# Gnnng/SVDFeature

Hardware: AMD Instinct MI355X
Metric: training instances/sec (SGD updates/s), basicMF k=64 (higher is better)
Workload: dtype f32; 1 GPU; basicMF synthetic 1000000x100000, 100000000 ratings, k=64 fp32 (BASELINE configs[1]); order=uniform random (file order preserved: result == sequential SGD), conflict_free_batches_per_pass=903, parallelism=1 GPU

## Files before the change

svdfeature_amd/csrc/svdf_capi.cpp:

```cpp
#include <svdfeature_amd.h>

#include <algorithm>
#include <cstdlib>
#include <cstring>
#include <new>
#include <vector>

#include "svdf_engine.h"
#include "svdf_kernels.h"
#include "svdf_wseq_rule.h"

namespace svdf {
void rank_eval_metrics(long S, const int64_t *sec_ptr, const int *position, const int *ranked, const int *nan, int num_at, const int *at,
                       svdf_rank_metrics *out);
void set_error_mode(int m);
const char *last_error();
void note_error(const std::string &m);
}

struct svdf_trainer { svdf::Engine *e; };
struct svdf_dataset { svdf::Dataset *d; };
struct svdf_ranker { svdf::Ranker *r; };

#define SVDF_GUARD(retval, ...)                                 \
// ... 212 lines not shown
int svdf_rank_prefetch_buffer_file(svdf_trainer *t, const char *path) { SVDF_GUARD(-1, { t->e->rank_prefetch(path); return 0; }) }
int64_t svdf_rank_sample_buffer_file(svdf_trainer *t, const char *in_path, const char *out_path) {
    SVDF_GUARD(-1, { return (int64_t)t->e->rank_sample_buffer_file(in_path, out_path); })
}
void svdf_dataset_destroy(svdf_dataset *ds) {
    if (!ds) return;
    try { if (ds->d && ds->d->owner) ds->d->owner->synchronize(); } catch (...) {}
    delete ds->d;
    delete ds;
}
int svdf_train_dataset(svdf_trainer *t, svdf_dataset *ds) { SVDF_GUARD(-1, { t->e->train_dataset(ds->d); return 0; }) }
int svdf_predict_dataset(svdf_trainer *t, svdf_dataset *ds, float *out) { SVDF_GUARD(-1, { t->e->predict_dataset(ds->d, out); return 0; }) }
int64_t svdf_dataset_info(const svdf_dataset *ds, int what) {
    if (!ds || !ds->d) return -1;
    switch (what) {
    case 0: return ds->d->num_row;
    case 1: return ds->d->kind == 8 ? (int64_t)ds->d->wchild.size() : (int64_t)ds->d->sched.num_levels();
    case 2: return ds->d->sched.max_level_size;
    case 3: return ds->d->kind;
    case 4: return ds->d->algorithmic_bytes;
    case 5: return ds->d->num_units;
    case 6: return ds->d->num_simple_units;
    case 7: {
        uint64_t h = 1469598103934665603ull;
        auto mix = [&h](uint64_t v) { for (int b = 0; b < 8; b++) { h ^= (v >> (8 * b)) & 0xFFu; h *= 1099511628211ull; } };
        for (long v : ds->d->sched.level_ptr) mix((uint64_t)v);
        for (long v : ds->d->sched.level_mid) mix((uint64_t)v);
        for (int v : ds->d->sched.order) mix((uint64_t)(unsigned)v);
        return (int64_t)(h >> 1);
    }
    case 8: return ds->d->kind == 8 && !ds->d->wchild.empty() ? (int64_t)ds->d->wchild[0]->kind : -1;
    case 9: return ds->d->rn_stage_state;
    case 10: return ds->d->rn_stage_bytes;
    default: return -1;
    }
}

int svdf_item_delta_begin(svdf_trainer *t) { SVDF_GUARD(-1, { t->e->per_rank_api(); t->e->item_delta_begin(); return 0; }) }
void *svdf_item_delta_buffer(svdf_trainer *t, int64_t *count) { SVDF_GUARD(nullptr, { t->e->per_rank_api(); return t->e->item_delta_buffer(count); }) }
int svdf_item_delta_apply(svdf_trainer *t) { SVDF_GUARD(-1, { t->e->per_rank_api(); t->e->item_delta_apply(); return 0; }) }
int svdf_item_delta_export(svdf_trainer *t, float *dst) { SVDF_GUARD(-1, { t->e->per_rank_api(); t->e->item_delta_copy(dst, nullptr); return 0; }) }
int svdf_item_delta_import(svdf_trainer *t, const float *src) { SVDF_GUARD(-1, { t->e->per_rank_api(); t->e->item_delta_copy(nullptr, src); return 0; }) }

int svdf_item_delta_into(svdf_trainer *t, float *dst, int64_t *count) { SVDF_GUARD(-1, { t->e->per_rank_api(); t->e->item_delta_into(dst, count); return 0; }) }
int svdf_item_delta_pack(svdf_trainer *t, void *dst, int half, int64_t *count) { SVDF_GUARD(-1, { t->e->per_rank_api(); t->e->item_delta_pack(dst, half, count); return 0; }) }
int svdf_item_delta_unpack(svdf_trainer *t, const void *src, int half, int refresh_snapshot) {
    SVDF_GUARD(-1, { t->e->per_rank_api(); t->e->item_delta_unpack(src, half, refresh_snapshot); return 0; })
}
int svdf_item_delta_select(svdf_trainer *t, int part, int nparts) { SVDF_GUARD(-1, { t->e->per_rank_api(); t->e->item_delta_select(part, nparts); return 0; }) }
int svdf_item_delta_apply_from(svdf_trainer *t, const float *src) { SVDF_GUARD(-1, { t->e->per_rank_api(); t->e->item_delta_apply_from(src); return 0; }) }
int svdf_set_stream(svdf_trainer *t, void *hip_stream) { SVDF_GUARD(-1, { t->e->set_stream((hipStream_t)hip_stream); return 0; }) }

int64_t svdf_get_view(svdf_trainer *t, int which, float *out, int64_t capacity) { SVDF_GUARD(-1, { return t->e->get_view(which, out, capacity); }) }
int64_t svdf_set_view(svdf_trainer *t, int which, const float *in, int64_t count) { SVDF_GUARD(-1, { return t->e->set_view(which, in, count); }) }
int svdf_view_shape(svdf_trainer *t, int which, int *rows, int *cols) { SVDF_GUARD(-1, { t->e->view_shape(which, rows, cols); return 0; }) }
void *svdf_stream(svdf_trainer *t) { return (void *)t->e->stream(); }
int svdf_synchronize(svdf_trainer *t) { SVDF_GUARD(-1, { t->e->synchronize(); return 0; }) }
int64_t svdf_counter(svdf_trainer *t, int what) { return t->e->counter(what); }
int svdf_set_knob(svdf_trainer *t, const char *name, long value) { SVDF_GUARD(-1, { return t->e->set_knob(name, value); }) }

int svdf_eval_dataset(svdf_trainer *t, svdf_dataset *ds, float scale_score, double *sum_sq_err, int64_t *count) {
    SVDF_GUARD(-1, { t->e->eval_dataset(ds->d, scale_score, sum_sq_err, count); return 0; })
}

int svdf_rank_eval_positions(svdf_trainer *t, long num_section, const unsigned *user, const int64_t *pos_ptr, const unsigned *pos_item,
                             const int64_t *ban_ptr, const unsigned *ban_item, int *position_out, int *tied_out, int *ranked_out, int *nan_out) {
// ... 117 lines not shown
```

svdfeature_amd/csrc/svdf_config.cpp:

```cpp
#include "svdf_engine.h"

#include <algorithm>
#include <chrono>
#include <cmath>
#include <cstdlib>
#include <cstring>
#include <memory>
#include <mutex>
#include <atomic>
#include <thread>

#include "svdf_kernels.h"
#include "svdf_internal.h"

namespace svdf {

void ParamSet::set_param(const char *name, const char *val) {
    if (!strncmp(name, prefix_a.c_str(), prefix_a.size())) name += prefix_a.size();
    else if (!strncmp(name, prefix_b.c_str(), prefix_b.size())) name += prefix_b.size();
    else return;
    if (!strcmp("bound", name)) {
        unsigned bd = (unsigned)atoi(val);
        check(bd > 0, "can't give 0 as bound");
        check(bound.empty() || bound.back() < bd, "bound must be given in order");
// ... 182 lines not shown
    case 38: return n_rank_eval_sections_;
    case 39: return n_rank_topn_sections_;
    case 21: return 0;
    default: return -1;
    }
}
int Engine::set_knob(const char *name, long value) {
    launch_version_++;
    if (multi_ && !is_peer_ && strcmp(name, "stage_window") != 0 && strcmp(name, "async_flush") != 0)
        for (int d = 1; d < gpus_; d++) (void)rank_engine(d)->set_knob(name, value);
    if (!strcmp(name, "use_graph")) { use_graph_ = value != 0; return 0; }
    if (!strcmp(name, "stage_window")) { check(value >= 1, "stage_window must be >= 1"); stage_window_ = value; window_set_ = true; return 0; }
    if (!strcmp(name, "groups_per_wave")) {
        check(value >= 0 && value <= 8 && value != 7, "groups_per_wave must be 0 (auto), 1 ... 6 or 8");
        groups_per_wave_ = (int)value;
        return 0;
    }
    if (!strcmp(name, "xcd_remap")) { xcd_remap_ = value != 0; params_dirty_ = true; return 0; }
    if (!strcmp(name, "fewrow_i16")) { check(value >= 0 && value <= 1, "fewrow_i16 must be 0 or 1"); fewrow_i16_ = (int)value; params_dirty_ = true; return 0; }
    if (!strcmp(name, "svdpp_helpers")) { check(value == 1 || value == 4 || value == 8 || value == 16, "svdpp_helpers must be 1, 4, 8 or 16"); svdpp_helpers_ = (int)value; params_dirty_ = true; return 0; }
    if (!strcmp(name, "basic_i8")) { check(value >= 0 && value <= 1, "basic_i8 must be 0 or 1"); basic_i8_ = (int)value; params_dirty_ = true; return 0; }
    if (!strcmp(name, "load_mode")) { check(value >= 0 && value <= 2, "load_mode must be 0, 1 or 2 (auto)"); load_mode_ = (int)value; params_dirty_ = true; return 0; }
    if (!strcmp(name, "store_mode")) { check(value >= 0 && value <= 2, "store_mode must be 0, 1 or 2"); store_mode_ = (int)value; params_dirty_ = true; return 0; }
    if (!strcmp(name, "sort_batches")) { check(value >= 0 && value <= 2, "sort_batches must be 0, 1 (by item) or 2 (by user)"); sort_batches_ = (int)value; return 0; }
    if (!strcmp(name, "async_flush")) { flush(); async_flush_ = value != 0; return 0; }
    if (!strcmp(name, "use_fused")) { use_fused_ = value != 0; return 0; }
    if (!strcmp(name, "device_schedule")) { device_sched_ = value != 0; return 0; }
    if (!strcmp(name, "device_rank")) { device_rank_ = value != 0; return 0; }
    if (!strcmp(name, "device_init")) { device_init_ = value != 0; return 0; }
    if (!strcmp(name, "device_window")) { device_window_ = value != 0; return 0; }
    if (!strcmp(name, "device_load")) { device_load_ = value != 0; return 0; }
    if (!strcmp(name, "runs_exec")) { check(value == 0 || value == 1, "runs_exec must be 0 or 1"); runs_exec_ = (int)value; return 0; }
    if (!strcmp(name, "runs_len")) { check(value >= 2 && value <= 7, "runs_len must be in 2 .. 7"); runs_len_ = (int)value; return 0; }
    if (!strcmp(name, "runs_sets")) { check(value >= 1 && value <= 2, "runs_sets must be 1 or 2"); runs_sets_ = (int)value; return 0; }
    if (!strcmp(name, "runs_block")) { check(value == 64 || value == 128 || value == 256, "runs_block must be 64, 128 or 256"); runs_block_ = (int)value; return 0; }
    if (!strcmp(name, "runs_min_rows")) { check(value >= 0, "runs_min_rows must not be negative"); runs_min_rows_ = value; return 0; }
    if (!strcmp(name, "runs_stage")) { check(value == 0 || value == 1, "runs_stage must be 0 or 1"); runs_stage_ = (int)value; return 0; }
    if (!strcmp(name, "runs_stage_max_mb")) { check(value >= -1, "runs_stage_max_mb must be -1 (no cap) or a size in MB"); runs_stage_max_mb_ = value; return 0; }
    if (!strcmp(name, "pair_units")) { check(value == 0 || value == 1, "pair_units must be 0 or 1"); pair_units_ = (int)value; return 0; }
    if (!strcmp(name, "pair_unit_cap")) { check(value >= 1 && value <= 4096, "pair_unit_cap must be in 1 .. 4096"); pair_unit_cap_ = (int)value; return 0; }
    if (!strcmp(name, "pivot_exec")) { check(value == 0 || value == 1, "pivot_exec must be 0 or 1"); pivot_exec_ = (int)value; return 0; }
    if (!strcmp(name, "pivot_run")) { check(value >= 1 && value <= 65536, "pivot_run must be in 1 .. 65536"); pivot_run_ = (int)value; return 0; }
    if (!strcmp(name, "pivot_min")) { check(value >= 2, "pivot_min must be at least 2"); pivot_min_ = (int)value; return 0; }
    if (!strcmp(name, "ipc_spin_limit")) { ipc_set_spin_limit(value); return 0; }
    if (!strcmp(name, "chain_width")) { check(value >= 0, "chain_width must not be negative"); chain_width_ = value; return 0; }
    if (!strcmp(name, "device_init_margin_log2")) { check(value >= 8 && value <= 52, "device_init_margin_log2 must be in 8 .. 52"); device_init_margin_log2_ = (int)value; return 0; }
    if (!strcmp(name, "device_schedule_min")) { check(value >= 1, "device_schedule_min must be >= 1"); device_sched_min_ = value; return 0; }
    if (!strcmp(name, "use_simple_units")) { use_simple_units_ = value != 0; return 0; }
    if (!strcmp(name, "rows_without_feedback")) { rows_without_feedback_ = value != 0; return 0; }
    if (!strcmp(name, "fewrow_gslots")) { fewrow_gslots_ = value != 0; launch_version_++; return 0; }
    if (!strcmp(name, "staged_pool")) { check(value == 0 || value == 1, "staged_pool must be 0 or 1"); flush(); staged_pool_mode_ = (int)value; return 0; }
    if (!strcmp(name, "wunit_inplace")) { wunit_inplace_ = value != 0; return 0; }
    if (!strcmp(name, "wunit_defer_fb")) { wunit_defer_fb_ = value != 0; return 0; }
    if (!strcmp(name, "wunit_fast")) { check(value >= 0 && value <= 3, "wunit_fast must be 0, 1, 2 or 3"); wunit_fast_ = (int)value; return 0; }
    if (!strcmp(name, "window_per_target_child")) { check(value >= 1, "window_per_target_child must be positive"); wseq_per_target_child_ = (int)value; return 0; }
    if (!strcmp(name, "window_per_target_shared")) { check(value >= 1, "window_per_target_shared must be positive"); wseq_per_target_shared_ = (int)value; return 0; }
    if (!strcmp(name, "window_per_target_fb")) { check(value >= 1, "window_per_target_fb must be positive"); wseq_per_target_fb_ = (int)value; return 0; }
    if (!strcmp(name, "window_shared_sub")) { check(value >= 0 && value <= 4096, "window_shared_sub must be in 0 .. 4096"); wseq_shared_sub_ = (int)value; return 0; }
    if (!strcmp(name, "window_shared_max")) { check(value >= 1, "window_shared_max must be positive"); wseq_shared_max_ = (int)value; return 0; }
    if (!strcmp(name, "window_item_sub")) { check(value >= 0 && value <= 128, "window_item_sub must be in 0 .. 128"); wseq_item_sub_ = (int)value; return 0; }
    if (!strcmp(name, "window_item_max")) { check(value >= 1, "window_item_max must be positive"); wseq_item_max_ = (int)value; return 0; }
    if (!strcmp(name, "window_block_sub")) {
        check(value >= 0 && value <= 4096, "window_block_sub must be in 0 .. 4096");
        check(value == 0 || (gpus_ == 1 && !multi_ && !is_peer_),
              "window_block_sub > 0 (ordered sub-steps for hot shared user rows of SVD++ blocks) is for the one-GPU window sequence; the N-rank exchange (amd:gpus > 1) has no place for user rows");
        wseq_block_sub_ = (int)value;
// ... 38 lines not shown
```

svdfeature_amd/csrc/svdf_dataset.cpp:

```cpp
#include "svdf_engine.h"

#include <algorithm>
#include <chrono>
#include <cmath>
#include <cstdlib>
#include <cstring>
#include <memory>
#include <mutex>
#include <atomic>
#include <thread>

#include "svdf_kernels.h"
#include "svdf_internal.h"

namespace svdf {

Dataset *Engine::dataset_from_blocks(long num_block, const int *extend_tag, const int64_t *fb_ptr, const unsigned *fb_index, const float *fb_value,
                                     const int64_t *block_row_ptr, const float *row_label, const int64_t *row_ptr, const unsigned *feat_index,
                                     const float *feat_value) {
    check(trainer_ready_, "dataset: init_trainer has not been called");
    need_device("dataset");
    check(user_group(), "svdfeature_amd: block datasets are for user-group (format_type 1) trainers");
    if (multi_ && !in_multi_scope()) {
        check(mp_.common_feedback_space == 0, "svdfeature_amd: amd:gpus > 1 needs a feedback space of its own (common_feedback_space = 0)");
// ... 534 lines not shown
    return true;
}
Dataset *Engine::auto_step(Dataset *exact, bool window_ok, const std::function<Dataset *()> &build_window) {
    std::unique_ptr<Dataset> ex(exact);
    AutoDecision D;
    double unit_us = 4.5;
    const bool from_probe = !ex;
    if (from_probe) { D = auto_probe_; D.decided = 0; }
    else auto_measures(ex.get(), D.levels, unit_us, D.dag_ms, D.stream_ms, pivot_run_);
    const bool deep = D.dag_ms > 2.0 * D.stream_ms;
    const char *why;
    if (!deep) { D.decided = 1; why = "exact levels kept (wide enough to stream)"; }
    else if (!window_ok) { D.decided = 3; why = "exact levels kept: the dependency depth binds, but the window step does not cover this configuration / these rows"; }
    else { D.decided = 2; why = "window step chosen: the dependency depth of exact sequential semantics binds"; }
    Dataset *out = ex.get();
    if (D.decided == 2) {
        ex.reset();
        out = build_window();
        D.windows = (long)out->wchild.size();
    } else {
        ex.release();
    }
    auto_last_ = D;
    if (!getenv("SVDF_QUIET"))
        fprintf(stderr, "[svdfeature_amd] amd:step = auto: %ld rows, %s%ld conflict-free levels: dag bound %.2f ms, stream model %.2f ms -> %s%s\n",
                (long)out->num_row, from_probe ? "extrapolated from the first 2 M rows: ~" : "", D.levels, D.dag_ms, D.stream_ms, why,
                D.decided == 2 ? (" (" + std::to_string(D.windows) + " windows)").c_str() : "");
    return out;
}

std::string Engine::path_for(const Dataset *ds) const {
    const DevParams &P = const_cast<Engine *>(this)->params();
    const long L = (long)ds->sched.num_levels();
    char buf[512];
    auto levels = [&](const char *what) { snprintf(buf, sizeof(buf), "exact, %ld conflict-free levels: %s", L, what); return std::string(buf); };
    switch (ds->kind) {
    case 0: return levels(chain_width_ > 0 ? "contract kernel k_basicmf / k_basicmf_slots, one (user, item) instance per lane group; narrow levels chained (k_basicmf_slots_chain)"
                                           : "contract kernel k_basicmf / k_basicmf_slots, one (user, item) instance per lane group");
    case 1: return levels("general sparse kernel k_general (any number of ids per row, side tables, lazy decay)");
    case 2: {
        const FusedSchedule S = ds->fused.view();
        if (fewrow_gslots_ && fewrow_fast_ && fewrow_gslots_applies(P, S, ds->fused.max_nu, ds->fused.max_ni, ds->fused.dense_slots))
            return levels("few-row kernel with global ids k_fewrow_gslots (neighbourhood shape)");
        return levels(fewrow_fast_ && fewrow_fast_applies(P, S) ? "few-row kernel k_fewrow_slots (<= 2 user + 2 item rows per instance: rank pairs, side ids); narrow levels chained"
                                                                 : "fused few-row kernel k_fused");
    }
    case 3: snprintf(buf, sizeof(buf), "exact, %ld conflict-free levels of user units: k_svdpp_wave (one wave per user, %ld of %ld units) + k_svdpp (general units)",
                     L, ds->num_simple_units, ds->num_units); return buf;
    case 4: return levels("multi-level implicit feedback units k_imfb");
    case 5: return "window data set (one window of the window-minibatch step, user side exact): k_window_users / k_window_items";
    case 6: return "amd:gpus handle: per-rank windows (svdf_multi.cpp)";
    case 7: return "window data set of user units: k_wunit_* (svdf_k_wunit.hip)";
    case 8: snprintf(buf, sizeof(buf), "window sequence (amd:step = minibatch / auto): %zu windows, each trained and applied in place%s%s; NOT the reference's sequential semantics (|dRMSE| <= 1e-4 contract)",
                     ds->wchild.size(), side_tables() ? ", feature_user / feature_item children as shared rows (general walk k_wunit_walk)" : "",
                     !ds->wchild.empty() && ds->wchild[0]->kind == 7 && !wunit_width_ok() ? ", user units of wide rows: the wide general walk k_wunit_walk<64, ., ., WideRow>, one wave per unit" : ""); return buf;
    case 9: snprintf(buf, sizeof(buf), "exact, %ld levels: hot rows walked as units (k_svdpp_wave on %s parameters, %ld units) + cold ratings through the contract kernel",
                     L, ds->pv_item_pivot ? "transposed" : "plain", ds->num_units); return buf;
    case 10: {
        char st[96] = "rows in W";
        if (runs_staged(ds)) snprintf(st, sizeof(st), "rows handed from run to run through staging slots (runs_stage, %.1f MB)", (double)ds->rn_stage_bytes / 1048576.0);
        else if (ds->rn_stage_state == 2) snprintf(st, sizeof(st), "rows in W (operand staging refused)");
        snprintf(buf, sizeof(buf), "exact, %ld levels of runs: k_basicmf_runs_soa (up to %d consecutive ratings of one item per lane group, the item's row in registers); %s", L, ds->rn_len, st);
        return buf;
    }
    case 11: snprintf(buf, sizeof(buf), "exact, %ld levels of user-run units: k_pair_units (%ld units of up to %d consecutive pairs of one user, the user's row in registers)",
                      L, ds->num_units, pair_unit_cap_); return buf;
    default: return "unknown";
    }
}
void Engine::note_dataset(Dataset *ds) {
    if (!ds || host_only_ || is_peer_) return;
    const bool verbose = getenv("SVDF_VERBOSE") != nullptr, quiet = getenv("SVDF_QUIET") != nullptr;
    if (verbose && !quiet) fprintf(stderr, "[svdfeature_amd] data set of %ld rows -> %s\n", (long)ds->num_row, path_for(ds).c_str());
    if (step_auto_set_ || step_minibatch_set_ || multi_ || gpus_ != 1) return;
    if (!(ds->kind == 0 || ds->kind == 1 || ds->kind == 2 || ds->kind == 3 || ds->kind == 4 || ds->kind == 9 || ds->kind == 10 || ds->kind == 11) || ds->num_row <= 0) return;
    AutoDecision D;
    double unit_us = 4.5;
    auto_measures(ds, D.levels, unit_us, D.dag_ms, D.stream_ms, pivot_run_);
    guard_last_ = D;
    if (D.dag_ms <= 10.0 * D.stream_ms || D.dag_ms < 50.0) return;
    n_guard_warnings_++;
    if (quiet) return;
    const bool window_ok = ds->plain_rows ? wunit_config_ok(false) && window_rows_allowed() && (wseq_pair_sub_ == 0 || wunit_width_ok())
                                          : wunit_config_ok() && (ds->kind == 3 || ds->kind == 4 || basic_fast_path_allowed());
    fprintf(stderr, "[svdfeature_amd] default (exact) step: %ld rows in %ld conflict-free levels -- the data's dependency depth binds: about %.0f ms per pass "
                    "(%.2f M rows/s; levels x %.1f us) against %.1f ms if the rows streamed.  The exact pass keeps the reference's sequential result bit for bit; "
                    "%s\n",
            (long)ds->num_row, D.levels, D.dag_ms, (double)ds->num_row / D.dag_ms * 1e-3, unit_us, D.stream_ms,
            window_ok ? "`amd:step = auto` would train this data set with the window step (user side exact, shared rows once per window; |dRMSE| <= 1e-4 contract) near the streaming rate"
                      : "the window step of `amd:step = auto` does not cover this configuration");
}

Dataset::~Dataset() {
    for (auto &per_rank : mchild) for (Dataset *c : per_rank) delete c;
    for (Dataset *c : wchild) delete c;
// ... 227 lines not shown
```

svdfeature_amd/csrc/svdf_engine.h:

```cpp
#ifndef SVDF_ENGINE_H_
#define SVDF_ENGINE_H_

#include <hip/hip_runtime.h>

#include <condition_variable>
#include <cstdio>
#include <memory>
#include <mutex>
#include <stdexcept>
#include <thread>
#include <string>
#include <deque>
#include <functional>
#include <future>
#include <map>
#include <vector>

#include "svdf_types.h"

namespace svdf {

struct Error : std::runtime_error {
    explicit Error(const std::string &m) : std::runtime_error(m) {}
};
// ... 196 lines not shown
    DevBuf<int> pos_list, neg_list;
    bool general = false;
    std::vector<int> h_tag;
    std::vector<int64_t> h_fb_ptr;
    std::vector<unsigned> h_fb_index;
    std::vector<float> h_fb_value;
    DevBuf<int> g_row_ptr, pair_p, pair_n, lens, optr;
    DevBuf<unsigned> g_index, out_index;
    DevBuf<float> g_value, out_label, out_value;
    void *scan_tmp = nullptr;
    size_t scan_tmp_bytes = 0;
    ~RankSource() { if (scan_tmp) (void)hipFree(scan_tmp); }
};
class Engine;
class Ranker;

struct Dataset {
    Engine *owner = nullptr;
    long num_row = 0;
    int kind = 0;
    DevBuf<WinUser> win_urec;
    DevBuf<int> win_slot, win_iptr, win_slot1;
    DevBuf<unsigned> win_item1;
    DevBuf<float> win_ival1;
    long win_item_lo = 0, win_item_hi = -1;
    DevBuf<long> d_level_ptr;
    bool d_level_ptr_ok = false;
    DevBuf<PairUnit> pu_units;
    DevBuf<unsigned> pu_lo, pu_hi;
    DevBuf<float> pu_vlo, pu_one;
    DevBuf<unsigned> rn_item, rn_user[8];
    DevBuf<float> rn_label[8];
    int rn_len = 0;
    DevBuf<float> rn_stage_row, rn_stage_bias;
    DevBuf<unsigned> rn_dst, rn_first;
    int rn_stage_state = 0;
    unsigned rn_stage_row0 = 0;
    int64_t rn_stage_bytes = 0;
    std::vector<long> pv_unit_ptr;
    bool pv_item_pivot = false;
    long pv_cold = 0, pv_hot_rows = 0;
    int64_t chained_levels = 0;
    bool win_hot = false;
    long win_slots = 0;
    DevBuf<int> win_pos;
    bool win_has_pos = false;
    std::vector<long> wfirst;
    DevBuf<WinUnit> wu_units;
    DevBuf<WinSeg> wu_segs;
    DevBuf<int> wu_rptr, wu_tptr, wu_gptr;
    DevBuf<WinEnt> wu_ent, wu_fbent;
    DevBuf<WinTouched> wu_touched;
    long wu_ntouched = -1;
    DevBuf<WinFbRec> wu_fbrec;
    long wu_nseg = 0;
    bool wu_defer_fb = false;
    long wu_gslots = 0;
    int wu_estride = 0;
    bool wu_feedback = false;
    DevBuf<int> wu_uptr, wu_upos;
    DevBuf<WinEnt> wu_uent;
    long wu_nshared = 0;
    bool wu_shared_uniform = false;
    DevBuf<int> wu_iptr;
    DevBuf<WinEnt> wu_ient;
    bool wu_ichild = false;
// ... 352 lines not shown
    int wseq_shared_sub_ = 0;
    int wseq_shared_max_ = 512;
    int wseq_item_sub_ = 0;
    int wseq_item_max_ = 2048;
    int wseq_block_sub_ = 0;
    int wseq_block_max_ = 512;
    int block_sub() const { return user_group() && shared_user() ? wseq_block_sub_ : 0; }
    void wseq_block_check(const char *what) const;
    int wseq_block_item_sub_ = 0;
    int wseq_block_item_max_ = 2048;
    int block_item_sub() const { return user_group() ? wseq_block_item_sub_ : 0; }
    void wseq_block_item_check(const char *what) const;
    int wseq_pair_sub_ = 0;
    int wseq_pair_max_ = 4096;
    int wseq_hot_sub_ = 128;
    int wseq_hot_max_ = 2048;
    DevBuf<float> d_clabel_;
    int wseq_count_actual_ = 1;
    WseqKnobs wseq_knobs() const;
    bool wseq_hot_ok() const;
    void wseq_pair_check(const char *what) const;
    void wseq_sub_check(const char *what, const char *knob, const char *desc, const char *entry, const char *nrank, bool entry_only = false) const;
    std::vector<long> wseq_item_counts(long n, const unsigned *item, const unsigned *item1) const;
    Dataset *wseq_from_columns(long n, const unsigned *user, const unsigned *item, const unsigned *item1, const float *label,
                               const std::vector<long> &item_count, WseqLane lane);
    void wseq_count_targets(WseqCounts &C, long r0, long r1, const int64_t *row_ptr, const unsigned *feat_index) const;
    void wseq_adopt_window(Dataset *ds, const WUnitHost &H, long first);
    int wseq_per_target_ = 24;
    bool single_minibatch() const { return step_minibatch_set_ && gpus_ == 1 && !multi_ && !is_peer_; }
    int runs_exec_ = 1;
    int runs_len_ = 4;
    int runs_sets_ = 1, runs_block_ = 64;
    long runs_min_rows_ = 1 << 20;
    int64_t n_runs_passes_ = 0;
    bool runs_config_ok() const;
    Dataset *runs_dataset_from_triples(long n, const unsigned *user, const unsigned *item, const float *label);
    void runs_train(Dataset *ds);
    int runs_stage_ = 1;
    long runs_stage_max_mb_ = -1;
    void runs_stage_build(Dataset *ds);
    bool runs_staged(const Dataset *ds) const { return runs_stage_ != 0 && ds->rn_stage_state == 1 && ds->rn_stage_row0 == user_off_; }
    int pivot_exec_ = 1;
    int pivot_run_ = 256, pivot_run_long_ = 256;
    int pivot_min_ = 2048;
    int64_t n_pivot_passes_ = 0;
    int pair_units_ = 1, pair_unit_cap_ = 16;
    int64_t n_punit_passes_ = 0;
    bool punit_config_ok() const;
    Dataset *punit_dataset_from_pairs(long n, const unsigned *user, const unsigned *pos, const unsigned *neg);
    bool punit_build(long n, const unsigned *user, const unsigned *lo, const unsigned *hi, std::vector<PairUnit> &sorted, std::vector<long> &level_ptr) const;
    bool punit_flush(HostCSR &src);
    DevBuf<PairUnit> w_pu_units_;
    PairUnitSchedule punit_view(const Dataset *ds) const;
    void punit_train(Dataset *ds);
    void punit_predict(Dataset *ds, float *d_out);
    bool pivot_config_ok() const;
    Dataset *pivot_dataset_from_triples(long n, const unsigned *user, const unsigned *item, const float *label);
    void pivot_train(Dataset *ds);
    bool step_auto_set_ = false, auto_building_ = false;
    struct AutoDecision { int decided = 0; long levels = 0, windows = 0; double dag_ms = 0.0, stream_ms = 0.0; } auto_last_;
    bool auto_step_active() const { return step_auto_set_ && !auto_building_ && gpus_ == 1 && !multi_ && !is_peer_ && !host_only_; }
    Dataset *auto_step(Dataset *exact, bool window_ok, const std::function<Dataset *()> &build_window);
    static constexpr long AUTO_PROBE_ROWS = 2000000, AUTO_PROBE_MIN = 8000000;
    AutoDecision auto_probe_;
    std::string auto_rank_path_;
    int auto_rank_decision_ = 0;
    bool auto_probe_deep(Dataset *probe, long n_full);
// ... 181 lines not shown
```

svdfeature_amd/csrc/svdf_k_runs.hip:

```cpp
#include "svdf_device.h"

namespace svdf {

__global__ __launch_bounds__(256) void k_runs_check(const unsigned *user, const unsigned *item, long n, unsigned nu, unsigned ni, unsigned *flag) {
    const long stride = (long)gridDim.x * blockDim.x;
    unsigned bad = 0u;
    for (long p = (long)blockIdx.x * blockDim.x + threadIdx.x; p < n; p += stride) {
        if (user[p] >= nu) bad |= 1u;
        if (item[p] >= ni) bad |= 2u;
    }
    if (bad) atomicOr(flag, bad);
}
__global__ __launch_bounds__(256) void k_runs_prev(const unsigned *keys, const unsigned *pos, long n, unsigned *prev) {
    const long stride = (long)gridDim.x * blockDim.x;
    for (long j = (long)blockIdx.x * blockDim.x + threadIdx.x; j < n; j += stride)
        prev[pos[j]] = (j > 0 && keys[j - 1] == keys[j]) ? pos[j - 1] : 0xFFFFFFFFu;
}
__global__ __launch_bounds__(256) void k_runs_form(const unsigned *ikeys, const unsigned *ipos, long n, unsigned num_item, const unsigned *prev, int R,
                                                   unsigned *head, unsigned *head_of, unsigned char *idx) {
    const long stride = (long)gridDim.x * blockDim.x;
    for (long it = (long)blockIdx.x * blockDim.x + threadIdx.x; it < (long)num_item; it += stride) {
        long lo = 0, hi = n;
        while (lo < hi) { const long mid = (lo + hi) >> 1; if (ikeys[mid] < (unsigned)it) lo = mid + 1; else hi = mid; }
        unsigned h = 0u;
// ... 23 lines not shown
    }
}
__global__ __launch_bounds__(256) void k_runs_fill_u32(unsigned *v, long n, unsigned x) {
    const long stride = (long)gridDim.x * blockDim.x;
    for (long j = (long)blockIdx.x * blockDim.x + threadIdx.x; j < n; j += stride) v[j] = x;
}
static inline int runs_grid(long n) { long g = (n + 255) / 256; return (int)(g < 1 ? 1 : (g > 16384 ? 16384 : g)); }
void launch_runs_check(const unsigned *user, const unsigned *item, long n, unsigned nu, unsigned ni, unsigned *flag, hipStream_t st) {
    if (n > 0) hipLaunchKernelGGL(k_runs_check, dim3(runs_grid(n)), dim3(256), 0, st, user, item, n, nu, ni, flag);
}
void launch_runs_prev(const unsigned *keys, const unsigned *pos, long n, unsigned *prev, hipStream_t st) {
    if (n > 0) hipLaunchKernelGGL(k_runs_prev, dim3(runs_grid(n)), dim3(256), 0, st, keys, pos, n, prev);
}
void launch_runs_form(const unsigned *ikeys, const unsigned *ipos, long n, unsigned num_item, const unsigned *prev, int R, unsigned *head, unsigned *head_of,
                      unsigned char *idx, hipStream_t st) {
    if (n > 0 && num_item > 0) hipLaunchKernelGGL(k_runs_form, dim3(runs_grid((long)num_item)), dim3(256), 0, st, ikeys, ipos, n, num_item, prev, R, head, head_of, idx);
}
void launch_runs_fill(const unsigned *user, const unsigned *item, const float *label, long n, const unsigned *unit_at, const unsigned *head_of,
                      const unsigned char *idx, long nunit, unsigned *c_item, unsigned *c_user, float *c_label, hipStream_t st) {
    if (n > 0) hipLaunchKernelGGL(k_runs_fill, dim3(runs_grid(n)), dim3(256), 0, st, user, item, label, n, unit_at, head_of, idx, nunit, c_item, c_user, c_label);
}
__global__ __launch_bounds__(256) void k_runs_iota(unsigned *v, long n) {
    const long stride = (long)gridDim.x * blockDim.x;
    for (long j = (long)blockIdx.x * blockDim.x + threadIdx.x; j < n; j += stride) v[j] = (unsigned)j;
}
void launch_runs_iota(unsigned *v, long n, hipStream_t st) {
    if (n <= 0) return;
    long grid = (n + 255) / 256;
    if (grid > 16384) grid = 16384;
    hipLaunchKernelGGL(k_runs_iota, dim3((int)grid), dim3(256), 0, st, v, n);
}
void launch_runs_fill_u32(unsigned *v, long n, unsigned x, hipStream_t st) {
    if (n > 0) hipLaunchKernelGGL(k_runs_fill_u32, dim3(runs_grid(n)), dim3(256), 0, st, v, n, x);
}

__global__ __launch_bounds__(256) void k_runs_inverse(const int *order, long nunit, unsigned *pos_of) {
    const long stride = (long)gridDim.x * blockDim.x;
    for (long s = (long)blockIdx.x * blockDim.x + threadIdx.x; s < nunit; s += stride) pos_of[order[s]] = (unsigned)s;
}
__global__ __launch_bounds__(256) void k_runs_operands(const RunSchedule S, const unsigned *pos_of, long nunit, int R, unsigned num_user, unsigned *keys, unsigned *vals) {
    const long stride = (long)gridDim.x * blockDim.x, m = nunit * (1 + R);
    for (long t = (long)blockIdx.x * blockDim.x + threadIdx.x; t < m; t += stride) {
        const long un = t / (1 + R);
        const int j = (int)(t - un * (1 + R));
        const unsigned s = pos_of[un];
        const unsigned id = j == 0 ? num_user + S.item[s] : S.user[j - 1][s];
        keys[t] = (j > 0 && id == (unsigned)SLOT_ABSENT) ? 0xFFFFFFFFu : id;
        vals[t] = (unsigned)((long)j * nunit + s);
    }
}
__global__ __launch_bounds__(256) void k_runs_links(const unsigned *keys, const unsigned *vals, long m, unsigned row0, unsigned *dst, unsigned *first) {
    const long stride = (long)gridDim.x * blockDim.x;
    for (long t = (long)blockIdx.x * blockDim.x + threadIdx.x; t < m; t += stride) {
        const unsigned key = keys[t], slot = vals[t];
        if (key == 0xFFFFFFFFu) { dst[slot] = (unsigned)SLOT_ABSENT; continue; }
        dst[slot] = (t + 1 < m && keys[t + 1] == key) ? vals[t + 1] : ((unsigned)RUNS_HOME | (row0 + key));
        if (t == 0 || keys[t - 1] != key) first[key] = slot;
    }
}
void launch_runs_stage_links(const RunSchedule &S, const int *order, long nunit, int R, unsigned num_user, unsigned row0, unsigned *pos_of, unsigned *ka, unsigned *kb,
                             unsigned *va, unsigned *vb, void **tmp, size_t *tmp_bytes, unsigned *dst, unsigned *first, long nrow, hipStream_t st) {
    if (nunit <= 0) return;
    const long m = nunit * (1 + R);
    hipLaunchKernelGGL(k_runs_inverse, dim3(runs_grid(nunit)), dim3(256), 0, st, order, nunit, pos_of);
    hipLaunchKernelGGL(k_runs_operands, dim3(runs_grid(m)), dim3(256), 0, st, S, pos_of, nunit, R, num_user, ka, va);
    device_sort_pairs_u32(ka, kb, va, vb, m, tmp, tmp_bytes, st);
// ... 188 lines not shown
```

svdfeature_amd/csrc/svdf_kernels.h:

```cpp
#ifndef SVDF_KERNELS_H_
#define SVDF_KERNELS_H_

#include <hip/hip_runtime.h>

#include <type_traits>
#include <vector>

#include "svdf_types.h"

namespace svdf {

int lanes_per_instance(int k);
int max_supported_factor();
int max_fast_path_factor();

void launch_basicmf(const DevParams &P, const BasicSchedule &S, long begin, long end, int groups_per_wave, int block_threads, hipStream_t st);
bool launch_basicmf_chain(const DevParams &P, const BasicSchedule &S, const long *d_level_ptr, long l0, long l1, hipStream_t st);
void launch_fused(const DevParams &P, const FusedSchedule &S, int max_nu, int max_ni, long begin, long end, int groups_per_wave,
                  int block_threads, hipStream_t st);
bool fewrow_fast_applies(const DevParams &P, const FusedSchedule &S);
bool launch_fewrow_chain(const DevParams &P, const FusedSchedule &S, int max_nu, int max_ni, const long *d_level_ptr, long l0, long l1, hipStream_t st);
bool fewrow_gslots_applies(const DevParams &P, const FusedSchedule &S, int max_nu, int max_ni, bool dense_slots);
void launch_fewrow_gslots(const DevParams &P, const FusedSchedule &S, long begin, long end, hipStream_t st);
void launch_fewrow_fast(const DevParams &P, const FusedSchedule &S, int max_nu, int max_ni, long begin, long end, int block_threads, hipStream_t st);
// ... 56 lines not shown
#define RANK_TILE 32
struct RankTile { int nsec; int off[RANK_TILE], nu[RANK_TILE], npos[RANK_TILE], nban[RANK_TILE], pos0[RANK_TILE]; };
void launch_rank_tile_open(const DevParams &P, const unsigned *stage, const RankTile &T, const float *fb_in, float *tuT, unsigned *banmask,
                           const unsigned *prev_ban, int nprev, int *cnt, unsigned *flag, long cap, const float *ifT, const float *ibias, float *pos_score,
                           unsigned *zero_words, long nzero, hipStream_t st);
void launch_rank_score_tile(const DevParams &P, long n, long cap, const float *tuT, const float *ifT, const float *ibias, const unsigned *banmask, unsigned *out,
                            const unsigned *stage, const RankTile &T, const float *pos_score, int *cnt, int mode, unsigned *wmin, unsigned *flag, hipStream_t st);
struct RselSecs { unsigned K1[RANK_TILE]; };
long rank_tile_minima(long n);
bool rank_tile_select_applies(long n, long cap, long K1max);
void launch_rank_tile_select(long n, long cap, int nsec, const unsigned *keys, const unsigned *wmin, const RselSecs &Ks, unsigned *out, long out_stride,
                             const unsigned *flag, hipStream_t st);
void launch_rank_select_tile(long n, long cap, int nsec, const unsigned *keys, const RselSecs &Ks, unsigned *work, unsigned *ck, unsigned *cv, unsigned *out,
                             long out_stride, unsigned *flag, hipStream_t st);
void launch_rank_positions(long n, const float *score, const signed char *tag, const int *pos_item, int npos, int *greater, int *ties, hipStream_t st);
long rank_select_work_words();
long rank_select_cap();
void launch_rank_select(long n, const unsigned *keys, const unsigned *vals, unsigned K1, unsigned *work, unsigned *ck, unsigned *cv, unsigned *out,
                        const unsigned *flag, hipStream_t st);
long device_exclusive_scan_u32(const unsigned *in, unsigned *out, long n, void **tmp, size_t *tmp_bytes, hipStream_t st);
void launch_runs_check(const unsigned *user, const unsigned *item, long n, unsigned nu, unsigned ni, unsigned *flag, hipStream_t st);
void launch_runs_prev(const unsigned *keys, const unsigned *pos, long n, unsigned *prev, hipStream_t st);
void launch_runs_form(const unsigned *ikeys, const unsigned *ipos, long n, unsigned num_item, const unsigned *prev, int R, unsigned *head, unsigned *head_of,
                      unsigned char *idx, hipStream_t st);
void launch_runs_fill(const unsigned *user, const unsigned *item, const float *label, long n, const unsigned *unit_at, const unsigned *head_of,
                      const unsigned char *idx, long nunit, unsigned *c_item, unsigned *c_user, float *c_label, hipStream_t st);
bool pair_units_applies(const DevParams &P);
void launch_pair_units(const DevParams &P, const PairUnitSchedule &S, long begin, long end, float *out, hipStream_t st);
void launch_runs_iota(unsigned *v, long n, hipStream_t st);
void launch_runs_fill_u32(unsigned *v, long n, unsigned x, hipStream_t st);
void launch_runs_stage_links(const RunSchedule &S, const int *order, long nunit, int R, unsigned num_user, unsigned row0, unsigned *pos_of, unsigned *ka, unsigned *kb,
                             unsigned *va, unsigned *vb, void **tmp, size_t *tmp_bytes, unsigned *dst, unsigned *first, long nrow, hipStream_t st);
void launch_runs_stage_in(const DevParams &P, const unsigned *first, long nrow, unsigned row0, float *stage_row, float *stage_bias, hipStream_t st);
bool basicmf_runs_soa_applies(const DevParams &P);
void launch_basicmf_runs_soa(const DevParams &P, const RunSchedule &S, long begin, long end, int R, int G, int block_threads, hipStream_t st);
void device_sort_pairs_u32(unsigned *keys_in, unsigned *keys_out, unsigned *vals_in, unsigned *vals_out, long n, void **tmp, size_t *tmp_bytes, hipStream_t st);
int sqerr_partials_grid(long n);
void launch_sqerr_partials(const float *pred, const float *label, long n, float scale, double *partials, hipStream_t st);
struct RankSourceDev {
    long num_block, num_row;
    const long *block_row_ptr;
    const float *label, *uval, *ival;
    const unsigned *uidx, *iidx;
};
struct SamplerParams { float pos_lowerb, neg_upperb; int sample_num, sample_max; };
struct PairColumns { float *label, *uval, *v0, *v1; unsigned *uidx, *i0, *i1; };
struct RankRowsDev {
    long num_block, num_row;
    const long *block_row_ptr;
    const float *label;
    const int *row_ptr;
    const unsigned *index;
    const float *value;
};
struct GSamplerParams { float pos_lowerb, neg_upperb, gap; int sample_num, sample_max, method, method_raw, pointwise; };
void launch_gsample_counts(const RankRowsDev &S, const GSamplerParams &sp, int *scratch, long *draws, long *pairs, hipStream_t st);
void launch_gsample_pairs(const RankRowsDev &S, const GSamplerParams &sp, const long *draw_off, const long *pair_off, const unsigned *raw, int *pos_list,
                          int *neg_list, int *pair_p, int *pair_n, hipStream_t st);
void launch_gpair_sizes(const RankRowsDev &S, const GSamplerParams &sp, long npairs, const int *pair_p, const int *pair_n, int *lens, hipStream_t st);
void launch_gpair_write(const RankRowsDev &S, const GSamplerParams &sp, long npairs, const int *pair_p, const int *pair_n, const int *optr, float *olabel,
                        unsigned *oi, float *ov, hipStream_t st);
void device_exclusive_scan_i32(const int *in, int *out, long n, void **tmp, size_t *tmp_bytes, hipStream_t st);
void host_sort_by_label(const float *label, long n, int *ids);
void host_parallel_sort_scores(const float *score, int *ids, long n, int nthreads);
void launch_rand_expand(const unsigned *tables, long nchunks, long C, long D, unsigned *raw, hipStream_t st);
struct WBuildIn { long n; int pairs; const unsigned *user, *item, *neg; const float *label; long num_user, num_item; };
// ... 108 lines not shown
```

svdfeature_amd/csrc/svdf_runs.cpp:

```cpp
#include <algorithm>
#include <cstring>
#include <memory>

#include "svdf_engine.h"
#include "svdf_kernels.h"
#include "svdf_internal.h"

namespace svdf {

bool Engine::runs_config_ok() const {
    return runs_exec_ != 0 && !host_only_ && device_sched_ && !user_group() && basic_fast_path_allowed() && mtype_.extend_type == 0 && mtype_.active_type == ACT_LINEAR &&
           tp_.reg_method == 0 && mp_.user_nonnegative == 0 && mp_.no_user_bias == 0 && u_param_.bound.empty() && i_param_.bound.empty() && (mp_.num_factor == 64 || mp_.num_factor == 128) &&
           basic_i8_ != 0 && store_mode_ == 0;
}

Dataset *Engine::runs_dataset_from_triples(long n, const unsigned *user, const unsigned *item, const float *label) {
    if (!runs_config_ok() || n < runs_min_rows_ || n >= 0x7FFFFFF0L) return nullptr;
    const int RF = std::max(2, std::min(7, runs_len_));
    const int R = RF <= 2 ? 2 : (RF <= 4 ? 4 : 7);
    const unsigned NU = (unsigned)mp_.num_user, NI = (unsigned)mp_.num_item;
    std::unique_ptr<Dataset> ds(new Dataset());
    adopt(ds.get());
    ds->kind = 10; ds->num_row = n; ds->rn_len = R;
    ds->user.upload(user, (size_t)n, stream_);
    ds->item.upload(item, (size_t)n, stream_);
    ds->label.upload(label, (size_t)n, stream_);
    ds->unit_values = true;
    DevBuf<unsigned> flag, ka, kb, va, vb, prev, head, head_of, unit_at, c_item, c_user;
    DevBuf<unsigned char> idx;
    DevBuf<float> c_label;
    flag.reserve(4);
    HIPCHECK(hipMemsetAsync(flag.p, 0, 4 * sizeof(unsigned), stream_));
    launch_runs_check(ds->user.p, ds->item.p, n, NU, NI, flag.p, stream_);
    unsigned hflag = 0;
    HIPCHECK(hipMemcpyAsync(&hflag, flag.p, sizeof(unsigned), hipMemcpyDeviceToHost, stream_));
    HIPCHECK(hipStreamSynchronize(stream_));
    if (hflag & 1u) fail("user feature index exceed bound");
    if (hflag & 2u) fail("item feature index exceed bound");
    ka.reserve((size_t)n); kb.reserve((size_t)n); va.reserve((size_t)n); vb.reserve((size_t)n);
    prev.reserve((size_t)n); head.reserve((size_t)n); head_of.reserve((size_t)n); unit_at.reserve((size_t)n); idx.reserve((size_t)n);
    void *tmp = nullptr;
    size_t tmp_bytes = 0;
    struct FreeTmp { void *&p; ~FreeTmp() { if (p) (void)hipFree(p); } } free_tmp{tmp};
    HIPCHECK(hipMemcpyAsync(ka.p, ds->user.p, (size_t)n * sizeof(unsigned), hipMemcpyDeviceToDevice, stream_));
    launch_runs_iota(va.p, n, stream_);
    device_sort_pairs_u32(ka.p, kb.p, va.p, vb.p, n, &tmp, &tmp_bytes, stream_);
    launch_runs_prev(kb.p, vb.p, n, prev.p, stream_);
    HIPCHECK(hipMemcpyAsync(ka.p, ds->item.p, (size_t)n * sizeof(unsigned), hipMemcpyDeviceToDevice, stream_));
    launch_runs_iota(va.p, n, stream_);
    device_sort_pairs_u32(ka.p, kb.p, va.p, vb.p, n, &tmp, &tmp_bytes, stream_);
    launch_runs_form(kb.p, vb.p, n, NI, prev.p, RF, head.p, head_of.p, idx.p, stream_);
    const long nunit = device_exclusive_scan_u32(head.p, unit_at.p, n, &tmp, &tmp_bytes, stream_);
    HIPCHECK(hipGetLastError());
    c_item.reserve((size_t)nunit); c_user.reserve((size_t)R * (size_t)nunit); c_label.reserve((size_t)R * (size_t)nunit);
    launch_runs_fill_u32(c_user.p, (long)R * nunit, (unsigned)SLOT_ABSENT, stream_);
    HIPCHECK(hipMemsetAsync(c_label.p, 0, (size_t)R * (size_t)nunit * sizeof(float), stream_));
    launch_runs_fill(ds->user.p, ds->item.p, ds->label.p, n, unit_at.p, head_of.p, idx.p, nunit, c_item.p, c_user.p, c_label.p, stream_);
    HIPCHECK(hipGetLastError());
    HIPCHECK(hipStreamSynchronize(stream_));
    ka.release(); kb.release(); va.release(); vb.release(); prev.release(); head.release(); head_of.release(); unit_at.release(); idx.release();
    const unsigned *res[SVDF_SCHED_MAX_SLOTS];
    unsigned off[SVDF_SCHED_MAX_SLOTS], limit[SVDF_SCHED_MAX_SLOTS];
    const char *msg[SVDF_SCHED_MAX_SLOTS];
    res[0] = c_item.p; off[0] = NU; limit[0] = NI; msg[0] = "item feature index exceed bound";
    std::vector<DUCol> du{DUCol{c_item.p, &ds->rn_item}};
    std::vector<DFCol> df;
    for (int j = 0; j < R; j++) {
        res[1 + j] = c_user.p + (size_t)j * (size_t)nunit; off[1 + j] = 0u; limit[1 + j] = NU; msg[1 + j] = "user feature index exceed bound";
        du.push_back(DUCol{c_user.p + (size_t)j * (size_t)nunit, &ds->rn_user[j]});
        df.push_back(DFCol{c_label.p + (size_t)j * (size_t)nunit, &ds->rn_label[j]});
    }
    schedule_device_columns(ds.get(), nunit, 1 + R, res, off, limit, msg, sort_batches_ == 1 ? c_item.p : nullptr, NI, du, df);
    ds->num_units = nunit;
    ds->algorithmic_bytes = n * (8L * mp_.num_factor * 2 + 8 * 2 + 16 + 8 * 2);
    if (runs_stage_) runs_stage_build(ds.get());
    return ds.release();
}

namespace {
template <typename T>
bool try_reserve(DevBuf<T> &b, size_t n) {
    b.release();
    if (hipMalloc((void **)&b.p, (n ? n : 1) * sizeof(T)) != hipSuccess) { (void)hipGetLastError(); b.p = nullptr; return false; }
    b.cap = n ? n : 1;
    return true;
}
}
void Engine::runs_stage_build(Dataset *ds) {
    ds->rn_stage_state = 2;
    ds->rn_stage_bytes = 0;
    const long nunit = ds->num_units, nrow = (long)mp_.num_user + (long)mp_.num_item;
    const int R = ds->rn_len;
    const long m = (long)(1 + R) * nunit;
    if (nunit <= 0) return;
    const int64_t bytes = (int64_t)m * ((int64_t)pitch_ * 4 + 8) + (int64_t)nrow * 4;
    auto refuse = [&](const char *why) {
        ds->rn_stage_row.release(); ds->rn_stage_bias.release(); ds->rn_dst.release(); ds->rn_first.release();
        if (!getenv("SVDF_QUIET"))
            fprintf(stderr, "[svdfeature_amd] data set of %ld rows: no operand staging (%.1f MB: %s); its runs keep reading and writing W\n", (long)ds->num_row, (double)bytes / 1048576.0, why);
    };
    if (item_off_ != user_off_ + (unsigned)mp_.num_user || n_uiset_ >= 0x7FFFFFFFL) { refuse("W_user and W_item are not adjacent in W"); return; }
    if (m >= 0x7FFFFFFFL) { refuse("more than 2^31 slots"); return; }
    if (runs_stage_max_mb_ >= 0 && bytes > (int64_t)runs_stage_max_mb_ * 1048576) { refuse("above runs_stage_max_mb"); return; }
    size_t free_b = 0, total_b = 0;
    if (hipMemGetInfo(&free_b, &total_b) != hipSuccess) { (void)hipGetLastError(); refuse("hipMemGetInfo failed"); return; }
    if ((uint64_t)bytes > (uint64_t)free_b / 2) { refuse("more than half of the free device memory"); return; }
// ... 51 lines not shown
```

Baseline: 6.241 billion instances/s.

## Order runs within each level by run length then deal them across lane groups

```diff
diff --git a/svdfeature_amd/csrc/svdf_capi.cpp b/svdfeature_amd/csrc/svdf_capi.cpp
--- a/svdfeature_amd/csrc/svdf_capi.cpp
+++ b/svdfeature_amd/csrc/svdf_capi.cpp
@@ -268,6 +268,9 @@
     case 8: return ds->d->kind == 8 && !ds->d->wchild.empty() ? (int64_t)ds->d->wchild[0]->kind : -1;
     case 9: return ds->d->rn_stage_state;
     case 10: return ds->d->rn_stage_bytes;
+    case 11: return ds->d->kind == 10 ? ds->d->rn_wave_steps : -1;
+    case 12: return ds->d->kind == 10 ? ds->d->rn_mixed_sets : -1;
+    case 13: return ds->d->kind == 10 ? ds->d->rn_order : -1;
     default: return -1;
     }
 }
diff --git a/svdfeature_amd/csrc/svdf_config.cpp b/svdfeature_amd/csrc/svdf_config.cpp
--- a/svdfeature_amd/csrc/svdf_config.cpp
+++ b/svdfeature_amd/csrc/svdf_config.cpp
@@ -238,6 +238,7 @@
     if (!strcmp(name, "device_load")) { device_load_ = value != 0; return 0; }
     if (!strcmp(name, "runs_exec")) { check(value == 0 || value == 1, "runs_exec must be 0 or 1"); runs_exec_ = (int)value; return 0; }
     if (!strcmp(name, "runs_len")) { check(value >= 2 && value <= 7, "runs_len must be in 2 .. 7"); runs_len_ = (int)value; return 0; }
+    if (!strcmp(name, "runs_order")) { check(value == 0 || value == 1, "runs_order must be 0 (by item) or 1 (by run length, then item)"); runs_order_ = (int)value; return 0; }
     if (!strcmp(name, "runs_sets")) { check(value >= 1 && value <= 2, "runs_sets must be 1 or 2"); runs_sets_ = (int)value; return 0; }
     if (!strcmp(name, "runs_block")) { check(value == 64 || value == 128 || value == 256, "runs_block must be 64, 128 or 256"); runs_block_ = (int)value; return 0; }
     if (!strcmp(name, "runs_min_rows")) { check(value >= 0, "runs_min_rows must not be negative"); runs_min_rows_ = value; return 0; }
diff --git a/svdfeature_amd/csrc/svdf_dataset.cpp b/svdfeature_amd/csrc/svdf_dataset.cpp
--- a/svdfeature_amd/csrc/svdf_dataset.cpp
+++ b/svdfeature_amd/csrc/svdf_dataset.cpp
@@ -590,8 +590,8 @@
 std::string Engine::path_for(const Dataset *ds) const {
     const DevParams &P = const_cast<Engine *>(this)->params();
     const long L = (long)ds->sched.num_levels();
-    char buf[512];
-    auto levels = [&](const char *what) { snprintf(buf, sizeof(buf), "exact, %ld conflict-free levels: %s", L, what); return std::string(buf); };
+    char buf[768];
+    auto levels =[&](const char *what) { snprintf(buf, sizeof(buf), "exact, %ld conflict-free levels: %s", L, what); return std::string(buf); };
     switch (ds->kind) {
     case 0: return levels(chain_width_ > 0 ? "contract kernel k_basicmf / k_basicmf_slots, one (user, item) instance per lane group; narrow levels chained (k_basicmf_slots_chain)"
                                            : "contract kernel k_basicmf / k_basicmf_slots, one (user, item) instance per lane group");
@@ -618,7 +618,11 @@
         char st[96] = "rows in W";
         if (runs_staged(ds)) snprintf(st, sizeof(st), "rows handed from run to run through staging slots (runs_stage, %.1f MB)", (double)ds->rn_stage_bytes / 1048576.0);
         else if (ds->rn_stage_state == 2) snprintf(st, sizeof(st), "rows in W (operand staging refused)");
-        snprintf(buf, sizeof(buf), "exact, %ld levels of runs: k_basicmf_runs_soa (up to %d consecutive ratings of one item per lane group, the item's row in registers); %s", L, ds->rn_len, st);
+        char hist[160] = "";
+        for (int c = 1, at = 0; c <= ds->rn_len && at < (int)sizeof(hist) - 24; c++) at += snprintf(hist + at, sizeof(hist) - (size_t)at, "%s%ld", c > 1 ? " / " : "", (long)ds->rn_hist[c]);
+        snprintf(buf, sizeof(buf), "exact, %ld levels of runs: k_basicmf_runs_soa (up to %d consecutive ratings of one item per lane group, the item's row in registers); %s; "
+                 "a level's runs by %s (runs_order %d): runs_wave_steps %ld, runs_mixed_sets %ld, runs of 1 .. %d ratings: %s", L, ds->rn_len, st,
+                 ds->rn_order ? "length, then item" : "item", ds->rn_order, (long)ds->rn_wave_steps, (long)ds->rn_mixed_sets, ds->rn_len, hist);
         return buf;
     }
     case 11: snprintf(buf, sizeof(buf), "exact, %ld levels of user-run units: k_pair_units (%ld units of up to %d consecutive pairs of one user, the user's row in registers)",
diff --git a/svdfeature_amd/csrc/svdf_engine.h b/svdfeature_amd/csrc/svdf_engine.h
--- a/svdfeature_amd/csrc/svdf_engine.h
+++ b/svdfeature_amd/csrc/svdf_engine.h
@@ -252,6 +252,8 @@
     DevBuf<unsigned> rn_item, rn_user[8];
     DevBuf<float> rn_label[8];
     int rn_len = 0;
+    int rn_order = 0;
+    int64_t rn_wave_steps = 0, rn_mixed_sets = 0, rn_hist[8] = {0, 0, 0, 0, 0, 0, 0, 0};
     DevBuf<float> rn_stage_row, rn_stage_bias;
     DevBuf<unsigned> rn_dst, rn_first;
     int rn_stage_state = 0;
@@ -670,7 +672,9 @@
     int runs_len_ = 4;
     int runs_sets_ = 1, runs_block_ = 64;
     long runs_min_rows_ = 1 << 20;
+    int runs_order_ = 1;
     int64_t n_runs_passes_ = 0;
+    void runs_order_stats(Dataset *ds);
     bool runs_config_ok() const;
     Dataset *runs_dataset_from_triples(long n, const unsigned *user, const unsigned *item, const float *label);
     void runs_train(Dataset *ds);
diff --git a/svdfeature_amd/csrc/svdf_k_runs.hip b/svdfeature_amd/csrc/svdf_k_runs.hip
--- a/svdfeature_amd/csrc/svdf_k_runs.hip
+++ b/svdfeature_amd/csrc/svdf_k_runs.hip
@@ -79,6 +79,88 @@
 }
 void launch_runs_fill_u32(unsigned *v, long n, unsigned x, hipStream_t st) {
     if (n > 0) hipLaunchKernelGGL(k_runs_fill_u32, dim3(runs_grid(n)), dim3(256), 0, st, v, n, x);
+}
+
+__device__ __forceinline__ int runs_length(const RunSchedule &S, size_t at, int R) {
+    int len = 0;
+#pragma unroll
+    for (int j = 0; j < 8; j++)
+        if (j < R && S.user[j][at] != (unsigned)SLOT_ABSENT) len = j + 1;
+    return len;
+}
+__global__ __launch_bounds__(256) void k_runs_order_key(const unsigned *c_item, const unsigned *c_user, long nunit, int R, unsigned num_item, unsigned *key) {
+    const long stride = (long)gridDim.x * blockDim.x;
+    for (long un = (long)blockIdx.x * blockDim.x + threadIdx.x; un < nunit; un += stride) {
+        int len = 0;
+        for (int j = 0; j < R; j++)
+            if (c_user[(size_t)j * (size_t)nunit + (size_t)un] != (unsigned)SLOT_ABSENT) len = j + 1;
+        key[un] = (unsigned)(R - len) * num_item + c_item[un];
+    }
+}
+__global__ __launch_bounds__(256) void k_runs_order_deal(const int *order, int *out, const long *level_ptr, int nlev, long nunit, int ips) {
+    const long stride = (long)gridDim.x * blockDim.x;
+    for (long s = (long)blockIdx.x * blockDim.x + threadIdx.x; s < nunit; s += stride) {
+        int lo = 0, hi = nlev - 1;
+        while (lo < hi) { const int mid = (lo + hi + 1) >> 1; if (level_ptr[mid] <= s) lo = mid; else hi = mid - 1; }
+        const long begin = level_ptr[lo], nf = (level_ptr[lo + 1] - begin) / ips, p = s - begin;
+        long to = s;
+        if (p < nf * ips) {
+            const long q = p / ips;
+            const int x = (int)(q & 7);
+            long base = 0;
+            for (int y = 0; y < x; y++) base += (nf - y + 7) / 8;
+            to = begin + (base + (q >> 3)) * ips + p % ips;
+        }
+        out[to] = order[s];
+    }
+}
+void launch_runs_order_deal(const int *order, int *out, const long *level_ptr, int nlev, long nunit, int ips, hipStream_t st) {
+    if (nunit > 0 && nlev > 0) hipLaunchKernelGGL(k_runs_order_deal, dim3(runs_grid(nunit)), dim3(256), 0, st, order, out, level_ptr, nlev, nunit, ips);
+}
+__global__ __launch_bounds__(256) void k_runs_order_stats(const RunSchedule S, const long *level_ptr, int nlev, long nunit, int R, int ips, unsigned long long *tot) {
+    const long stride = (long)gridDim.x * blockDim.x;
+    const int lane = threadIdx.x & 63;
+    unsigned long long steps = 0ull, mixed = 0ull, cnt[8];
+#pragma unroll
+    for (int c = 0; c < 8; c++) cnt[c] = 0ull;
+    for (long base = (long)blockIdx.x * blockDim.x + (threadIdx.x & ~63); base < nunit; base += stride) {
+        const long s = base + lane;
+        const bool on = s < nunit;
+        int len = 0;
+        if (on) {
+            int lo = 0, hi = nlev - 1;
+            while (lo < hi) { const int mid = (lo + hi + 1) >> 1; if (level_ptr[mid] <= s) lo = mid; else hi = mid - 1; }
+            len = runs_length(S, (size_t)s, R);
+            const long begin = level_ptr[lo], end = level_ptr[lo + 1];
+            if ((s - begin) % ips == 0) {
+                int mx = len;
+                bool mix = false;
+                for (int t = 1; t < ips && s + t < end; t++) {
+                    const int l2 = runs_length(S, (size_t)(s + t), R);
+                    mix = mix || l2 != len;
+                    mx = l2 > mx ? l2 : mx;
+                }
+                steps += (unsigned long long)mx;
+                mixed += mix ? 1ull : 0ull;
+            }
+        }
+#pragma unroll
+        for (int c = 1; c < 8; c++) cnt[c] += (unsigned long long)__popcll(__ballot(on && len == c));
+    }
+    for (int o = 32; o > 0; o >>= 1) { steps += __shfl_xor(steps, o); mixed += __shfl_xor(mixed, o); }
+    if (lane == 0) {
+        if (steps) atomicAdd(tot, steps);
+        if (mixed) atomicAdd(tot + 1, mixed);
+#pragma unroll
+        for (int c = 1; c < 8; c++)
+            if (cnt[c]) atomicAdd(tot + 1 + c, cnt[c]);
+    }
+}
+void launch_runs_order_key(const unsigned *c_item, const unsigned *c_user, long nunit, int R, unsigned num_item, unsigned *key, hipStream_t st) {
+    if (nunit > 0) hipLaunchKernelGGL(k_runs_order_key, dim3(runs_grid(nunit)), dim3(256), 0, st, c_item, c_user, nunit, R, num_item, key);
+}
+void launch_runs_order_stats(const RunSchedule &S, const long *level_ptr, int nlev, long nunit, int R, int ips, unsigned long long *tot, hipStream_t st) {
+    if (nunit > 0 && nlev > 0) hipLaunchKernelGGL(k_runs_order_stats, dim3(runs_grid(nunit)), dim3(256), 0, st, S, level_ptr, nlev, nunit, R, ips, tot);
 }
 
 __global__ __launch_bounds__(256) void k_runs_inverse(const int *order, long nunit, unsigned *pos_of) {
diff --git a/svdfeature_amd/csrc/svdf_kernels.h b/svdfeature_amd/csrc/svdf_kernels.h
--- a/svdfeature_amd/csrc/svdf_kernels.h
+++ b/svdfeature_amd/csrc/svdf_kernels.h
@@ -112,6 +112,9 @@
 void launch_runs_stage_links(const RunSchedule &S, const int *order, long nunit, int R, unsigned num_user, unsigned row0, unsigned *pos_of, unsigned *ka, unsigned *kb,
                              unsigned *va, unsigned *vb, void **tmp, size_t *tmp_bytes, unsigned *dst, unsigned *first, long nrow, hipStream_t st);
 void launch_runs_stage_in(const DevParams &P, const unsigned *first, long nrow, unsigned row0, float *stage_row, float *stage_bias, hipStream_t st);
+void launch_runs_order_key(const unsigned *c_item, const unsigned *c_user, long nunit, int R, unsigned num_item, unsigned *key, hipStream_t st);
+void launch_runs_order_deal(const int *order, int *out, const long *level_ptr, int nlev, long nunit, int ips, hipStream_t st);
+void launch_runs_order_stats(const RunSchedule &S, const long *level_ptr, int nlev, long nunit, int R, int ips, unsigned long long *tot, hipStream_t st);
 bool basicmf_runs_soa_applies(const DevParams &P);
 void launch_basicmf_runs_soa(const DevParams &P, const RunSchedule &S, long begin, long end, int R, int G, int block_threads, hipStream_t st);
 void device_sort_pairs_u32(unsigned *keys_in, unsigned *keys_out, unsigned *vals_in, unsigned *vals_out, long n, void **tmp, size_t *tmp_bytes, hipStream_t st);
diff --git a/svdfeature_amd/csrc/svdf_runs.cpp b/svdfeature_amd/csrc/svdf_runs.cpp
--- a/svdfeature_amd/csrc/svdf_runs.cpp
+++ b/svdfeature_amd/csrc/svdf_runs.cpp
@@ -12,6 +12,33 @@
     return runs_exec_ != 0 && !host_only_ && device_sched_ && !user_group() && basic_fast_path_allowed() && mtype_.extend_type == 0 && mtype_.active_type == ACT_LINEAR &&
            tp_.reg_method == 0 && mp_.user_nonnegative == 0 && mp_.no_user_bias == 0 && u_param_.bound.empty() && i_param_.bound.empty() && (mp_.num_factor == 64 || mp_.num_factor == 128) &&
            basic_i8_ != 0 && store_mode_ == 0;
+}
+
+static constexpr bool runs_order_key_fits(int R, unsigned NI) { return (uint64_t)R * (uint64_t)NI <= 0xFFFFFFFFull; }
+static_assert(runs_order_key_fits(7, 1u << 27) && runs_order_key_fits(7, 613566756u) && !runs_order_key_fits(7, 613566757u), "R = 7: 7 * NI up to 2^32 - 1");
+static_assert(runs_order_key_fits(4, (1u << 30) - 1u) && !runs_order_key_fits(4, 1u << 30), "R = 4: NI below 2^30");
+static_assert(runs_order_key_fits(2, (1u << 31) - 1u) && !runs_order_key_fits(2, 1u << 31), "R = 2: NI below 2^31");
+
+void Engine::runs_order_stats(Dataset *ds) {
+    const long nunit = ds->num_units;
+    const size_t nlev = ds->sched.num_levels();
+    if (nunit <= 0 || nlev == 0 || nlev >= 0x7FFFFFFFul) return;
+    DevBuf<long> lp;
+    DevBuf<unsigned long long> tot;
+    lp.upload(ds->sched.level_ptr.data(), nlev + 1, stream_);
+    tot.reserve(9);
+    HIPCHECK(hipMemsetAsync(tot.p, 0, 9 * sizeof(unsigned long long), stream_));
+    RunSchedule S;
+    memset(&S, 0, sizeof(S));
+    for (int j = 0; j < ds->rn_len; j++) S.user[j] = ds->rn_user[j].p;
+    launch_runs_order_stats(S, lp.p, (int)nlev, nunit, ds->rn_len, mp_.num_factor == 128 ? 4 : 8, tot.p, stream_);
+    HIPCHECK(hipGetLastError());
+    unsigned long long h[9];
+    HIPCHECK(hipMemcpyAsync(h, tot.p, sizeof(h), hipMemcpyDeviceToHost, stream_));
+    HIPCHECK(hipStreamSynchronize(stream_));
+    ds->rn_wave_steps = (int64_t)h[0];
+    ds->rn_mixed_sets = (int64_t)h[1];
+    for (int c = 1; c < 8; c++) ds->rn_hist[c] = (int64_t)h[1 + c];
 }
 
 Dataset *Engine::runs_dataset_from_triples(long n, const unsigned *user, const unsigned *item, const float *label) {
@@ -70,8 +97,38 @@
         du.push_back(DUCol{c_user.p + (size_t)j * (size_t)nunit, &ds->rn_user[j]});
         df.push_back(DFCol{c_label.p + (size_t)j * (size_t)nunit, &ds->rn_label[j]});
     }
-    schedule_device_columns(ds.get(), nunit, 1 + R, res, off, limit, msg, sort_batches_ == 1 ? c_item.p : nullptr, NI, du, df);
+    const unsigned *sort_key = sort_batches_ == 1 ? c_item.p : nullptr;
+    unsigned sort_max = NI;
+    DevBuf<unsigned> c_key;
+    if (sort_batches_ == 1 && runs_order_ == 1 && runs_order_key_fits(R, NI)) {
+        c_key.reserve((size_t)nunit);
+        launch_runs_order_key(c_item.p, c_user.p, nunit, R, NI, c_key.p, stream_);
+        HIPCHECK(hipGetLastError());
+        sort_key = c_key.p; sort_max = (unsigned)R * NI;
+        ds->rn_order = 1;
+    }
+    if (ds->rn_order == 1) {
+        schedule_device_columns(ds.get(), nunit, 1 + R, res, off, limit, msg, sort_key, sort_max, {}, {});
+        const size_t nlev = ds->sched.num_levels();
+        if (nlev > 0 && nlev < 0x7FFFFFFFul) {
+            DevBuf<long> lp;
+            DevBuf<int> dealt;
+            lp.upload(ds->sched.level_ptr.data(), nlev + 1, stream_);
+            dealt.reserve((size_t)nunit);
+            launch_runs_order_deal(ds->order_dev.p, dealt.p, lp.p, (int)nlev, nunit, mp_.num_factor == 128 ? 4 : 8, stream_);
+            HIPCHECK(hipMemcpyAsync(ds->order_dev.p, dealt.p, (size_t)nunit * sizeof(int), hipMemcpyDeviceToDevice, stream_));
+            HIPCHECK(hipGetLastError());
+            HIPCHECK(hipStreamSynchronize(stream_));
+        }
+        for (const DUCol &c : du) { c.dst->reserve((size_t)nunit); device_gather_u32(c.src, ds->order_dev.p, c.dst->p, nunit, stream_); }
+        for (const DFCol &c : df) { c.dst->reserve((size_t)nunit); device_gather_f32(c.src, ds->order_dev.p, c.dst->p, nunit, stream_); }
+        HIPCHECK(hipGetLastError());
+        HIPCHECK(hipStreamSynchronize(stream_));
+    } else {
+        schedule_device_columns(ds.get(), nunit, 1 + R, res, off, limit, msg, sort_key, sort_max, du, df);
+    }
     ds->num_units = nunit;
+    runs_order_stats(ds.get());
     ds->algorithmic_bytes = n * (8L * mp_.num_factor * 2 + 8 * 2 + 16 + 8 * 2);
     if (runs_stage_) runs_stage_build(ds.get());
     return ds.release();
```

Result: faster. 6.477 billion instances/s (median of 6 runs) (+3.8%).
